# g1mv/density

Hardware: NVIDIA H100
Metric: chameleon_encode_input_GBps (higher is better)
Workload: dtype u32

## Files before the change

density_b200/csrc/api.cu:

```cuda
#include "../../include/density_b200.h"
#include "common.cuh"
#include "encode_internal.cuh"
#include "decode_bounds.cuh"

#include <dlfcn.h>

#include <atomic>
#include <condition_variable>
#include <cstdio>
#include <cstring>
#include <deque>
#include <mutex>
#include <string>
#include <thread>
#include <vector>

namespace dns {

static thread_local std::string g_last_error;
static std::atomic<uint64_t> g_launches{0};

static void set_error(const char* what, cudaError_t e) {
    char buf[512];
    snprintf(buf, sizeof buf, "%s: %s (%s)", what, cudaGetErrorString(e), cudaGetErrorName(e));
// ... 118 lines not shown
        ring.used[k] = true;
    }
    return e;
}
static cudaError_t d2h_any(PinRing& ring, uint8_t* dst, const uint8_t* src_dev, size_t n, cudaStream_t s, bool pageable) {
    if (!pageable) return cudaMemcpyAsync(dst, src_dev, n, cudaMemcpyDeviceToHost, s);
    cudaError_t e = ring.ensure();
    size_t pend_off = 0, pend_len = 0; unsigned pend_k = 0; bool pending = false;
    for (size_t off = 0; off < n && e == cudaSuccess; off += PIN_SLOT) {
        const size_t len = n - off < PIN_SLOT ? n - off : PIN_SLOT;
        const unsigned k = ring.next++ & 1u;
        if (ring.used[k] && !(pending && pend_k == k)) e = cudaEventSynchronize(ring.ev[k]);
        if (e != cudaSuccess) break;
        e = cudaMemcpyAsync(ring.slot[k], src_dev + off, len, cudaMemcpyDeviceToHost, s);
        if (e == cudaSuccess) e = cudaEventRecord(ring.ev[k], s);
        ring.used[k] = true;
        if (pending && e == cudaSuccess) {
            e = cudaEventSynchronize(ring.ev[pend_k]);
            if (e == cudaSuccess) CopyPool::get().copy(dst + pend_off, ring.slot[pend_k], pend_len);
        }
        pend_off = off; pend_len = len; pend_k = k; pending = true;
    }
    if (pending && e == cudaSuccess) {
        e = cudaEventSynchronize(ring.ev[pend_k]);
        if (e == cudaSuccess) CopyPool::get().copy(dst + pend_off, ring.slot[pend_k], pend_len);
    }
    return e;
}

struct DeviceCtx {
    int dev = -1;
    int num_sms = 0;
    bool ready = false;
    cudaStream_t stream = nullptr;
    cudaStream_t h2d_stream = nullptr, d2h_stream = nullptr;
    DevBuf ws, stage_in, stage_out, pipe_tables, dec_tables;
    DevBuf chee_tables[2][3];
    uint32_t chee_epoch = 0;
    uint64_t* h_sizes = nullptr;
    cudaEvent_t ev_h2d[2] = {nullptr, nullptr};
    PinRing ring_in, ring_out;
    uint64_t* d_size = nullptr;
    uint64_t* h_size = nullptr;
    ChamLayout layout{};
    int last_was_chameleon_fastpath_capable = 0;
    bool profile = false;
    static constexpr int PROF_RING = 64;
    cudaEvent_t ev[PROF_RING][4] = {};
    uint64_t prof_count = 0;
    const void* last_cl_status = nullptr;
    DevBuf lion_stats; bool lion_stats_valid = false;
    cudaEvent_t ws_free = nullptr;
    bool ws_free_recorded = false;
    std::mutex mu;
};

constexpr int MAX_DEVICES = 64;
static DeviceCtx g_ctx[MAX_DEVICES];
static std::mutex g_ctx_mu;

static DeviceCtx* current_ctx() {
    int dev = -1;
    cudaError_t e = cudaGetDevice(&dev);
    if (e != cudaSuccess) { set_error("cudaGetDevice", e); return nullptr; }
    if (dev < 0 || dev >= MAX_DEVICES) { set_error("device index out of range"); return nullptr; }
    DeviceCtx* c = &g_ctx[dev];
    std::lock_guard<std::mutex> lk(g_ctx_mu);
    if (!c->ready) {
        cudaDeviceProp prop;
        e = cudaGetDeviceProperties(&prop, dev);
        if (e != cudaSuccess) { set_error("cudaGetDeviceProperties", e); return nullptr; }
        if (prop.major != 9 || prop.minor != 0) { set_error("density_b200 is built for sm_90a and requires a compute capability 9.0 device (H100)"); return nullptr; }
        c->dev = dev;
        c->num_sms = prop.multiProcessorCount;
        e = cudaStreamCreateWithFlags(&c->stream, cudaStreamNonBlocking);
        if (e == cudaSuccess) e = cudaStreamCreateWithFlags(&c->h2d_stream, cudaStreamNonBlocking);
        if (e == cudaSuccess) e = cudaStreamCreateWithFlags(&c->d2h_stream, cudaStreamNonBlocking);
        if (e != cudaSuccess) { set_error("cudaStreamCreate", e); return nullptr; }
        e = cudaMalloc(&c->d_size, 64);
        if (e != cudaSuccess) { set_error("cudaMalloc", e); return nullptr; }
        e = cudaMallocHost(&c->h_size, 64);
        if (e == cudaSuccess) e = cudaMallocHost(&c->h_sizes, sizeof(uint64_t) * 4096);
        if (e != cudaSuccess) { set_error("cudaMallocHost", e); return nullptr; }
        e = cudaEventCreateWithFlags(&c->ws_free, cudaEventDisableTiming);
        if (e != cudaSuccess) { set_error("cudaEventCreate", e); return nullptr; }
        c->ready = true;
    }
    return c;
}

static size_t safe_size(int alg, size_t size) {
    const size_t B = alg_block_bytes(alg), S = alg_sig_bytes(alg);
    return size + (size / B) * S + ((size % B) ? S : 0);
}

static bool is_device_pointer(const void* p) {
    cudaPointerAttributes a;
    cudaError_t e = cudaPointerGetAttributes(&a, p);
    if (e != cudaSuccess) { cudaGetLastError(); return false; }
    return a.type == cudaMemoryTypeDevice || a.type == cudaMemoryTypeManaged;
}

static bool ws_acquire(DeviceCtx* c, cudaStream_t stream) {
    if (!c->ws_free_recorded) return true;
    cudaError_t e = cudaStreamWaitEvent(stream, c->ws_free, 0);
    if (e != cudaSuccess) { set_error("cudaStreamWaitEvent", e); return false; }
    return true;
}
static void ws_release(DeviceCtx* c, cudaStream_t stream) {
    if (cudaEventRecord(c->ws_free, stream) == cudaSuccess) c->ws_free_recorded = true;
}

static int encode_device_locked_impl(DeviceCtx* c, int alg, const uint8_t* d_in, size_t n, uint8_t* d_out, size_t cap,
                                     uint64_t* d_out_size, cudaStream_t stream, int path);
static int encode_device_locked(DeviceCtx* c, int alg, const uint8_t* d_in, size_t n, uint8_t* d_out, size_t cap,
                                uint64_t* d_out_size, cudaStream_t stream, int path) {
    if (!ws_acquire(c, stream)) return DENSITY_B200_ECUDA;
    const int rc = encode_device_locked_impl(c, alg, d_in, n, d_out, cap, d_out_size, stream, path);
    ws_release(c, stream);
    return rc;
}
static int encode_device_locked_impl(DeviceCtx* c, int alg, const uint8_t* d_in, size_t n, uint8_t* d_out, size_t cap,
                                     uint64_t* d_out_size, cudaStream_t stream, int path) {
    uint64_t launches = 0;
    cudaError_t e;
    const bool aligned = !(reinterpret_cast<uintptr_t>(d_in) & 3) && !(reinterpret_cast<uintptr_t>(d_out) & 1);
    if (alg == ALG_CHAMELEON && path != 3 && aligned) {
        ChamLayout L;
        size_t need = cham_workspace_bytes(n, c->num_sms, &L);
        e = c->ws.ensure(need, stream);
        if (e != cudaSuccess) { set_error("workspace cudaMalloc", e); return DENSITY_B200_ECUDA; }
        c->layout = L;
        if (path == 2) {
            e = cham_encode_protected_only(d_in, n, c->ws.p, L, d_out, cap, d_out_size, stream, &launches);
        } else {
            const uint32_t nruns = cham_pick_runs(n, c->num_sms);
            cudaEvent_t* ev = nullptr;
            if (c->profile) {
                ev = c->ev[c->prof_count % DeviceCtx::PROF_RING];
                for (int i = 0; i < 4; ++i) if (!ev[i]) cudaEventCreate(&ev[i]);
            }
            e = cham_encode_phase1(d_in, n, c->ws.p, L, nruns, nullptr, stream, &launches, ev);
            if (e == cudaSuccess && path == 4)
                e = cham_encode_phase2_blocking(d_in, n, c->ws.p, L, nruns, d_out, cap, d_out_size, 12, c->num_sms, stream, &launches);
            else if (e == cudaSuccess)
                e = cham_encode_phase2(d_in, n, c->ws.p, L, nruns, nullptr, d_out, cap, d_out_size, path == 0, false, c->num_sms, stream, &launches, ev);
            if (ev != nullptr && e == cudaSuccess) c->prof_count++;
        }
        c->last_was_chameleon_fastpath_capable = (path != 2);
    } else if ((alg == ALG_CHEETAH || alg == ALG_LION) && path != 3 && !(reinterpret_cast<uintptr_t>(d_in) & 3) && !(reinterpret_cast<uintptr_t>(d_out) & 1)) {
        const size_t pw = (chee_workspace_bytes(n, c->num_sms) + 255) & ~(size_t)255;
        e = c->ws.ensure(pw + 256 + scalar_workspace_bytes(alg), stream);
        if (e != cudaSuccess) { set_error("workspace cudaMalloc", e); return DENSITY_B200_ECUDA; }
        DevBuf* tb = c->chee_tables[alg == ALG_LION];
        for (int rg = 0; rg < 3 && e == cudaSuccess; ++rg) e = tb[rg].ensure(chee_tables_bytes(alg, rg, n, c->num_sms) + 256, stream);
        if (e != cudaSuccess) { set_error("workspace cudaMalloc", e); return DENSITY_B200_ECUDA; }
        if (c->chee_epoch > 0x0FFFFF00u) {
            for (int a2 = 0; a2 < 2; ++a2) for (int rg = 0; rg < 3; ++rg)
                if (c->chee_tables[a2][rg].p) { e = cudaMemsetAsync(c->chee_tables[a2][rg].p, 0, c->chee_tables[a2][rg].bytes, stream); if (e != cudaSuccess) break; }
            if (e != cudaSuccess) { set_error("cudaMemsetAsync", e); return DENSITY_B200_ECUDA; }
            c->chee_epoch = 0;
        }
        uint32_t* d_conv = reinterpret_cast<uint32_t*>(c->ws.p + pw);
        uint8_t* const tabs[3] = {tb[0].p, tb[1].p, tb[2].p};
        for (int attempt = 0; attempt <= (path == 4 ? 12 : 0); ++attempt) {
            if (attempt > 0) {
                uint32_t conv = 0;
                e = cudaMemcpyAsync(&conv, d_conv, sizeof conv, cudaMemcpyDeviceToHost, stream);
                if (e == cudaSuccess) e = cudaStreamSynchronize(stream);
                if (e != cudaSuccess || conv) break;
            }
            const uint32_t epoch_base = c->chee_epoch + 1;
            c->chee_epoch += 32;
            e = chee_encode_parallel(alg, d_in, n, d_out, cap, c->ws.p, tabs, epoch_base, c->num_sms, d_out_size, d_conv, attempt > 0, stream, &launches);
            if (e != cudaSuccess) break;
        }
        if (e == cudaSuccess && path != 1)
            e = scalar_encode(alg, d_in, n, d_out, cap, c->ws.p + pw + 256, d_out_size, stream, &launches, d_conv);
        c->last_was_chameleon_fastpath_capable = 0;
    } else {
        if (reinterpret_cast<uintptr_t>(d_out) & 1) { set_error("encode_device: d_out must be 2-byte aligned"); return DENSITY_B200_EARG; }
        e = c->ws.ensure(scalar_workspace_bytes(alg), stream);
        if (e != cudaSuccess) { set_error("workspace cudaMalloc", e); return DENSITY_B200_ECUDA; }
        e = scalar_encode(alg, d_in, n, d_out, cap, c->ws.p, d_out_size, stream, &launches);
        c->last_was_chameleon_fastpath_capable = 0;
    }
    return step_result(e, launches, "encode launch");
}

static int decode_device_locked_impl(DeviceCtx* c, int alg, const uint8_t* d_in, size_t n, uint8_t* d_out, size_t cap,
                                     uint64_t* d_out_size, cudaStream_t stream, int path);
static int decode_device_locked(DeviceCtx* c, int alg, const uint8_t* d_in, size_t n, uint8_t* d_out, size_t cap,
                                uint64_t* d_out_size, cudaStream_t stream, int path = 0) {
    if (!ws_acquire(c, stream)) return DENSITY_B200_ECUDA;
    const int rc = decode_device_locked_impl(c, alg, d_in, n, d_out, cap, d_out_size, stream, path);
    ws_release(c, stream);
    return rc;
}
static int decode_device_locked_impl(DeviceCtx* c, int alg, const uint8_t* d_in, size_t n, uint8_t* d_out, size_t cap,
// ... 1993 lines not shown
```

density_b200/csrc/chameleon_encode.cu:

```cuda
#include <cstdio>
#include "common.cuh"
#include "encode_internal.cuh"

namespace dns {
namespace cham {

constexpr int TILE_Q = 4096;
__device__ __forceinline__ bool bit_test(const uint32_t* bm, uint32_t i) { return (bm[i >> 5] >> (i & 31)) & 1u; }

constexpr int F6_THREADS = 512, F6_QPT = 8;
constexpr int F6_NW = F6_THREADS / 32, F6_WQ = 32 * F6_QPT;
static_assert(F6_THREADS * F6_QPT == TILE_Q, "tile geometry");
constexpr int F6_MB_SLOTS = 4096, F6_MB_CAP = 4;
constexpr int F6_SEC_SLOTS = 64, F6_SEC_CAP = 16;
#ifdef DNS_PHASE_TIMING
__device__ long long g_f6_ph[8];
#define F6_PH(k) { if (threadIdx.x == 0 && blockIdx.x == 77) { long long tn = clock64(); g_f6_ph[k] += tn - f6_tprev; f6_tprev = tn; } }
#define F6_PH_DECL long long f6_tprev = clock64();
#else
#define F6_PH(k)
#define F6_PH_DECL
#endif
constexpr uint32_t F6_TOUCHED = 1u << 12, F6_DROPPED = 1u << 13;
struct Flag6Smem {
    uint16_t tab[65536];
    uint32_t vbit[2048];
    uint2 rec[TILE_Q];
    union {
        uint16_t mb[F6_MB_SLOTS][F6_MB_CAP];
        uint2 stage[F6_NW][64];
    };
    uint32_t mbcnt[2][F6_MB_SLOTS / 4];
    __align__(16) uint32_t sec[F6_SEC_SLOTS][F6_SEC_CAP];
    uint32_t seccnt[2][F6_SEC_SLOTS];
    uint32_t sigw[2][TILE_Q / 32];
    uint32_t cnt[32];
    uint32_t unres_count;
    uint32_t overflow;
};
static_assert(sizeof(Flag6Smem) <= 227 * 1024, "flag pass shared memory");

__device__ __forceinline__ void f6_append_unres(bool pred, uint32_t qidx_in_run, uint32_t hf, uint32_t* s_count, uint2* __restrict__ unres_run) {
    const uint32_t m = __ballot_sync(0xFFFFFFFFu, pred);
    if (m == 0) return;
    uint32_t base = 0;
    if ((threadIdx.x & 31) == 0) base = atomicAdd(s_count, (uint32_t)__popc(m));
    base = __shfl_sync(0xFFFFFFFFu, base, 0);
    if (pred) {
        const uint32_t idx = base + __popc(m & lanemask_lt());
        if (idx < 65536u) unres_run[idx] = make_uint2(qidx_in_run, hf);
    }
}

// ... 1048 lines not shown
    for (uint32_t g = 0; g < ngrp; ++g) { gin[g] = x; if (x != PC_ESC) x = GT[(size_t)g * PC_NC + x]; }
    gin[ngrp] = x;
    if (x == PC_ESC) words[1] = 1;
}
__global__ void cham_prot_seams_k(uint32_t nseg, const Status* __restrict__ st, const uint16_t* __restrict__ T, const uint32_t* __restrict__ gin,
                                  uint32_t* __restrict__ in_state) {
    if (!gate_open(st)) return;
    const uint32_t ngrp = (nseg + PC_GROUP - 1) / PC_GROUP;
    const uint32_t g = blockIdx.x * blockDim.x + threadIdx.x;
    if (g >= ngrp || gin[ngrp] == PC_ESC) return;
    uint32_t x = gin[g];
    const uint32_t s1 = ((g + 1) * PC_GROUP < nseg) ? (g + 1) * PC_GROUP : nseg;
    for (uint32_t s = g * PC_GROUP; s < s1; ++s) { in_state[s] = x; x = T[(size_t)s * PC_NC + x]; }
}
__global__ void cham_prot_walk_k(uint64_t nblocks, uint32_t nseg, const Status* __restrict__ st, int it, int warm, const uint8_t* __restrict__ inc,
                                 const uint8_t* __restrict__ cm_old, uint8_t* __restrict__ cm_new, const uint32_t* __restrict__ in_state,
                                 const uint32_t* __restrict__ gin, ProtShard* __restrict__ ps, uint32_t* __restrict__ words) {
    if (!gate_open(st)) return;
    const uint32_t ngrp = (nseg + PC_GROUP - 1) / PC_GROUP;
    const uint32_t s = blockIdx.x * blockDim.x + threadIdx.x;
    if (s >= nseg || gin[ngrp] == PC_ESC) return;
    Protection p; pc_decode(in_state[s], p);
    const uint64_t b0 = (uint64_t)s * PSEG, b1 = (b0 + PSEG < nblocks) ? b0 + PSEG : nblocks;
    p.counter = ps->first_block + b0;
    prot_walk(p, inc, b0, b1, cm_new);
    uint32_t nd = 0;
    for (uint64_t b = b0; b < b1; ++b) nd += cm_new[b] != ((it || warm) ? cm_old[b] : 0);
    if (nd) {
        atomicAdd(&words[0], nd);
        if (it < 16) atomicAdd(&ps->changed[it], nd);
    }
}

__device__ __forceinline__ void prot_round_verdict(const uint32_t* all_words, uint32_t world, uint32_t stride, bool& changed, bool& esc) {
    changed = false; esc = false;
    for (uint32_t r = 0; r < world; ++r) { changed |= all_words[stride * r] != 0; esc |= all_words[stride * r + 1] != 0; }
}
__global__ void cham_prot_commit_k(const uint32_t* __restrict__ all_words, uint32_t world, uint32_t stride, uint64_t nblocks, const Status* __restrict__ st,
                                   int it, uint8_t* __restrict__ cm_old, const uint8_t* __restrict__ cm_new) {
    if (!gate_open(st)) return;
    bool changed, esc;
    prot_round_verdict(all_words, world, stride, changed, esc);
    if (esc || !(changed || it == 0)) return;
    for (uint64_t b = (uint64_t)blockIdx.x * blockDim.x + threadIdx.x; b < nblocks; b += (uint64_t)gridDim.x * blockDim.x) cm_old[b] = cm_new[b];
}
__global__ void cham_prot_verdict_k(const uint32_t* __restrict__ all_words, uint32_t world, uint32_t stride, Status* __restrict__ st, int it,
                                    ProtShard* __restrict__ ps) {
    if (threadIdx.x || blockIdx.x || !gate_open(st)) return;
    bool changed, esc;
    prot_round_verdict(all_words, world, stride, changed, esc);
    if (esc) { ps->esc = 1; st->converged = 1; }
    else if (!changed) { ps->settled = 1; ps->rounds = (uint32_t)it + 1; st->converged = 1; }
}
__global__ void cham_prot_finish_k(Status* __restrict__ st, const ProtShard* __restrict__ ps) {
    if (threadIdx.x || blockIdx.x) return;
    if (!ps->settled || !ps->stage_ok) st->error = PROT_REFUSED;
}
__global__ void cham_prot_seam_words_k(uint64_t nblocks, const Status* __restrict__ st, uint64_t* __restrict__ d_out_size, uint32_t* __restrict__ words) {
    if (threadIdx.x || blockIdx.x) return;
    const uint64_t sz = (nblocks && !st->error) ? *d_out_size : 0;
    *d_out_size = sz;
    words[0] = 0; words[1] = 0; words[2] = st->error ? 1u : 0u; words[3] = nblocks ? 1u : 0u;
    words[4] = (uint32_t)sz; words[5] = (uint32_t)(sz >> 32); words[6] = 0; words[7] = 0;
}

}

using namespace cham;

size_t cham_workspace_bytes(size_t nbytes, int nruns_max, ChamLayout* L) {
    const uint64_t nblocks = (nbytes + 255) / 256;
    const uint64_t ntiles = (nblocks + 63) / 64;
    const uint64_t ngroups = (ntiles + SCAN_G - 1) / SCAN_G;
    size_t off = 0;
    auto take = [&](size_t bytes) { size_t o = off; off += (bytes + 255) & ~(size_t)255; return o; };
    L->status = take(sizeof(Status));
    L->sigw = take((ntiles * 64 * 2 + 64 + 256) * sizeof(uint32_t));
    L->copymap = take(ntiles * 64 + 64 + 128);
    L->copymap2 = take(ntiles * 64 + 64 + 128);
    L->seg_state = take(prot_state_bytes(ntiles * 64 / PSEG + 2));
    L->incb = take(ntiles * 64 + 64);
    L->tile_bytes = take((ntiles + 1) * sizeof(uint32_t));
    L->tile_local = take((ntiles + 1) * sizeof(uint32_t));
    L->group_total = take((ngroups + 1) * sizeof(uint64_t));
    L->group_off = take((ngroups + 1) * sizeof(uint64_t));
    L->unres = take((size_t)nruns_max * 65536 * sizeof(uint2));
    L->unres_count = take((size_t)nruns_max * sizeof(uint32_t));
    L->final_tab = take((size_t)nruns_max * 65536 * sizeof(uint32_t));
    L->carry = take((size_t)nruns_max * 65536 * sizeof(uint32_t));
    L->total = off;
    return off;
}

static cudaError_t set_smem_attrs_once() {
    static bool done = false;
    static cudaError_t err = cudaSuccess;
    if (!done) {
        err = cudaFuncSetAttribute(cham_flag_pass6, cudaFuncAttributeMaxDynamicSharedMemorySize, (int)sizeof(Flag6Smem));
        if (err == cudaSuccess)
            err = cudaFuncSetAttribute(cham_protected_pass, cudaFuncAttributeMaxDynamicSharedMemorySize, (int)sizeof(ProtSmem));
        done = true;
    }
    return err;
}

static cudaError_t prot_iterate_coop(int ctas, cudaStream_t stream, const uint32_t* sigw, uint64_t nbytes, uint64_t nblocks, uint32_t nseg, Status* st, int it,
// ... 4 lines not shown

cudaError_t prot_debug_read(unsigned long long* out32) { return cudaMemcpyFromSymbol(out32, g_prot_dbg, sizeof(unsigned long long) * 32); }

size_t prot_state_bytes(uint64_t nseg_max) { return (2 * (nseg_max + 2) + 64) * sizeof(uint32_t) + prot_table_elems(nseg_max) * sizeof(uint16_t); }

uint32_t cham_pick_runs(size_t nbytes, int num_sms) {
    const uint64_t nblocks = (nbytes + 255) / 256;
    const uint64_t ntiles = (nblocks + 63) / 64;
    uint64_t r = ntiles / 16;
    if (r < 1) r = 1;
    if (r > (uint64_t)num_sms) r = num_sms;
    return (uint32_t)r;
}

struct ChamBufs {
    size_t nbytes; uint64_t nquads, nblocks; uint32_t ntiles, ngroups, nseg, ngrp;
    Status* st; uint32_t* sigw; uint8_t *copymap, *copymap2, *incb; uint32_t *seg_state, *tile_bytes, *tile_local; uint64_t *group_total, *group_off;
    uint2* unres; uint32_t *unres_count, *final_tab, *carry;
    uint32_t *in_state, *out_state, *gin; uint16_t *ptab, *T, *GT;
    template <class X> static X* at(uint8_t* ws, size_t off) { return reinterpret_cast<X*>(ws + off); }
    ChamBufs(uint8_t* ws, const ChamLayout& L, size_t n) {
        nbytes = n; nquads = n / 4; nblocks = (n + 255) / 256;
        ntiles = (uint32_t)((nblocks + 63) / 64); ngroups = (ntiles + SCAN_G - 1) / SCAN_G;
        nseg = (uint32_t)((nblocks + PSEG - 1) / PSEG); ngrp = (nseg + PC_GROUP - 1) / PC_GROUP;
        st = at<Status>(ws, L.status); sigw = at<uint32_t>(ws, L.sigw);
        copymap = ws + L.copymap; copymap2 = ws + L.copymap2; incb = ws + L.incb;
        seg_state = at<uint32_t>(ws, L.seg_state);
        tile_bytes = at<uint32_t>(ws, L.tile_bytes); tile_local = at<uint32_t>(ws, L.tile_local);
        group_total = at<uint64_t>(ws, L.group_total); group_off = at<uint64_t>(ws, L.group_off);
        unres = at<uint2>(ws, L.unres); unres_count = at<uint32_t>(ws, L.unres_count);
        final_tab = at<uint32_t>(ws, L.final_tab); carry = at<uint32_t>(ws, L.carry);
        in_state = seg_state; out_state = seg_state + (nseg + 1);
        ptab = reinterpret_cast<uint16_t*>(seg_state + 2 * (nseg + 1));
        gin = reinterpret_cast<uint32_t*>(ptab); T = ptab + 2 * (ngrp + 2); GT = T + (size_t)nseg * PC_NC;
    }
};

static void launch_flag_pass(const ChamBufs& B, const uint8_t* d_in, uint32_t nruns, const uint8_t* copymap, const Status* gate, cudaStream_t stream,
                             uint64_t* launches) {
    cham_flag_pass6<<<nruns, F6_THREADS, sizeof(Flag6Smem), stream>>>(reinterpret_cast<const uint32_t*>(d_in), B.nquads, B.ntiles, nruns, B.sigw, B.unres,
                                                                      B.unres_count, B.final_tab, copymap, gate);
    ++*launches;
}
static void launch_carry_resolve(const ChamBufs& B, uint32_t nruns, const uint32_t* d_carry_in, const Status* gate, cudaStream_t stream,
                                 uint64_t* launches) {
    cham_carry_scan<<<65536 / 256, 256, 0, stream>>>(B.final_tab, d_carry_in, 0, nruns, B.carry, nullptr, gate);
    cham_resolve<<<dim3(32, nruns), 256, 0, stream>>>(B.unres, B.unres_count, B.carry, B.ntiles, nruns, B.sigw, gate);
    *launches += 2;
}
static void launch_export_fold(const ChamBufs& B, uint32_t nruns, uint32_t* d_table_out, const Status* gate, cudaStream_t stream, uint64_t* launches) {
    cham_carry_scan<<<65536 / 256, 256, 0, stream>>>(B.final_tab, nullptr, 1, nruns, nullptr, d_table_out, gate);
    ++*launches;
}
static cudaError_t sizes_scan_emit(const ChamBufs& B, const uint8_t* d_in, const uint8_t* copymap, int use_copymap_if_nonquiet, bool al16_ok,
                                   uint8_t* d_out, size_t cap, uint64_t* d_out_size, cudaStream_t stream, uint64_t* launches, cudaEvent_t* ev) {
    if (copymap) {
        cham_tile_sizes<<<(B.ntiles + 7) / 8, 256, 0, stream>>>(B.sigw, copymap, B.nbytes, B.nblocks, B.ntiles, use_copymap_if_nonquiet, 0, 0, B.st, B.tile_bytes);
        ++*launches;
    }
    cudaError_t e = scan_tiles_launch(B.tile_bytes, B.ntiles, B.tile_local, B.group_total, B.group_off, B.ngroups, B.st, (uint64_t)cap, d_out_size, stream);
    if (e != cudaSuccess) return e;
    *launches += 2;
    if (ev) cudaEventRecord(ev[2], stream);
    const uint32_t* in32 = reinterpret_cast<const uint32_t*>(d_in);
    if (al16_ok && (reinterpret_cast<uintptr_t>(d_in) & 15u) == 0)
        cham_emit<true><<<B.ntiles, EM_THREADS, 0, stream>>>(in32, B.nbytes, B.nblocks, B.sigw, copymap, use_copymap_if_nonquiet, B.st, B.tile_local, B.group_off, d_out);
    else
        cham_emit<false><<<B.ntiles, EM_THREADS, 0, stream>>>(in32, B.nbytes, B.nblocks, B.sigw, copymap, use_copymap_if_nonquiet, B.st, B.tile_local, B.group_off, d_out);
    ++*launches;
    if (ev) cudaEventRecord(ev[3], stream);
    return cudaGetLastError();
}

cudaError_t cham_encode_phase1(const uint8_t* d_in, size_t nbytes, uint8_t* ws, const ChamLayout& L, uint32_t nruns,
                               uint32_t* d_table_out, cudaStream_t stream, uint64_t* launches, cudaEvent_t* ev) {
    cudaError_t e = set_smem_attrs_once();
    if (e != cudaSuccess) return e;
    const ChamBufs B(ws, L, nbytes);
    e = cudaMemsetAsync(B.st, 0, sizeof(Status), stream);
    if (e == cudaSuccess) e = cudaMemsetAsync(&B.st->first_nonquiet_block, 0xFF, sizeof(unsigned long long), stream);
    if (e != cudaSuccess) return e;
    if (B.nblocks == 0) return cudaSuccess;
    if (ev) cudaEventRecord(ev[0], stream);
    launch_flag_pass(B, d_in, nruns, nullptr, nullptr, stream, launches);
    if (ev) cudaEventRecord(ev[1], stream);
    if (d_table_out) launch_export_fold(B, nruns, d_table_out, nullptr, stream, launches);
    return cudaGetLastError();
}

static cudaError_t cham_phase2_begin(const ChamBufs& B, uint32_t nruns, const uint32_t* d_carry_in, bool assume_prev_inc, cudaStream_t stream,
                                     uint64_t* launches) {
    launch_carry_resolve(B, nruns, d_carry_in, nullptr, stream, launches);
    cham_tile_sizes<<<(B.ntiles + 7) / 8, 256, 0, stream>>>(B.sigw, nullptr, B.nbytes, B.nblocks, B.ntiles, 0, 1, assume_prev_inc ? 1 : 0, B.st, B.tile_bytes);
    ++*launches;
    return cudaGetLastError();
}

static cudaError_t cham_phase2_rounds(const ChamBufs& B, const uint8_t* d_in, uint32_t nruns, const uint32_t* d_carry_in, int it_first, int it_last,
                                      bool reset_barriers, int num_sms, cudaStream_t stream, uint64_t* launches) {
    const int num_ctas = num_sms > 0 ? num_sms : 1;
    if (it_last - it_first >= 8) return cudaErrorInvalidValue;
    if (reset_barriers) {
        cudaError_t e = cudaMemsetAsync(B.st->barrier, 0, sizeof(B.st->barrier), stream);
        if (e != cudaSuccess) return e;
    }
    for (int it = it_first; it <= it_last; ++it) {
        if (it > 0) {
            launch_flag_pass(B, d_in, nruns, B.copymap, B.st, stream, launches);
            launch_carry_resolve(B, nruns, d_carry_in, B.st, stream, launches);
        }
        cudaError_t le = prot_iterate_coop(num_ctas, stream, B.sigw, B.nbytes, B.nblocks, B.nseg, B.st, it, B.incb, B.copymap, B.copymap2, B.in_state,
                                           B.out_state, B.ptab);
        if (le != cudaSuccess) return le;
        ++*launches;
    }
    return cudaGetLastError();
}

static cudaError_t cham_phase2_finish(const ChamBufs& B, const uint8_t* d_in, uint8_t* d_out, size_t cap, uint64_t* d_out_size, bool with_copy_map,
                                      bool inorder_fallback, cudaStream_t stream, uint64_t* launches, cudaEvent_t* ev) {
    if (with_copy_map && inorder_fallback) {
        cham_protected_pass<<<1, 1024, sizeof(ProtSmem), stream>>>(reinterpret_cast<const uint32_t*>(d_in), B.nbytes, B.st, 1, B.sigw, B.copymap);
        ++*launches;
    }
    return sizes_scan_emit(B, d_in, with_copy_map ? B.copymap : nullptr, 1, true, d_out, cap, d_out_size, stream, launches, ev);
}

static cudaError_t cham_phase2_needs_more(const ChamBufs& B, cudaStream_t stream, bool* more) {
    Status h;
    cudaError_t e = cudaMemcpyAsync(&h, B.st, sizeof h, cudaMemcpyDeviceToHost, stream);
    if (e == cudaSuccess) e = cudaStreamSynchronize(stream);
    if (e != cudaSuccess) return e;
    *more = h.nonquiet && !h.converged && !h.error;
    return cudaSuccess;
}

constexpr int PROT_ITERS = 4;

struct Phase2Opts {
    const uint32_t* d_carry_in = nullptr;
    bool assume_prev_inc = false;
    bool iterate = true;
    int max_batches = 0;
    bool inorder_walk = true;
    bool* give_up = nullptr;
    uint32_t* d_table_out = nullptr;
    cudaEvent_t* ev = nullptr;
};

static cudaError_t cham_phase2(const uint8_t* d_in, size_t nbytes, uint8_t* ws, const ChamLayout& L, uint32_t nruns, uint8_t* d_out, size_t cap,
                               uint64_t* d_out_size, const Phase2Opts& o, int num_sms, cudaStream_t stream, uint64_t* launches) {
    if (nbytes == 0) return cudaMemsetAsync(d_out_size, 0, sizeof(uint64_t), stream);
    const ChamBufs B(ws, L, nbytes);
    cudaError_t e = cham_phase2_begin(B, nruns, o.d_carry_in, o.assume_prev_inc, stream, launches);
    if (e == cudaSuccess && o.iterate) e = cham_phase2_rounds(B, d_in, nruns, o.d_carry_in, 0, PROT_ITERS, false, num_sms, stream, launches);
    bool more = false;
    const int looks = o.max_batches + (o.give_up ? 1 : 0);
    for (int batch = 0; e == cudaSuccess && batch < looks; ++batch) {
        e = cham_phase2_needs_more(B, stream, &more);
        if (e != cudaSuccess || !more || batch >= o.max_batches) break;
        e = cham_phase2_rounds(B, d_in, nruns, o.d_carry_in, 8, 15, true, num_sms, stream, launches);
    }
    if (e != cudaSuccess) return e;
    if (o.give_up && more) { *o.give_up = true; return cudaSuccess; }
    e = cham_phase2_finish(B, d_in, d_out, cap, d_out_size, o.iterate, o.inorder_walk, stream, launches, o.ev);
    if (e == cudaSuccess && o.d_table_out) {
        launch_export_fold(B, nruns, o.d_table_out, nullptr, stream, launches);
        e = cudaGetLastError();
    }
    return e;
}

cudaError_t cham_encode_phase2(const uint8_t* d_in, size_t nbytes, uint8_t* ws, const ChamLayout& L, uint32_t nruns,
                               const uint32_t* d_carry_in, uint8_t* d_out, size_t cap, uint64_t* d_out_size,
                               bool allow_protected_fallback, bool assume_prev_inc, int num_sms, cudaStream_t stream, uint64_t* launches,
                               cudaEvent_t* ev) {
    Phase2Opts o;
    o.d_carry_in = d_carry_in; o.assume_prev_inc = assume_prev_inc; o.iterate = allow_protected_fallback; o.ev = ev;
    return cham_phase2(d_in, nbytes, ws, L, nruns, d_out, cap, d_out_size, o, num_sms, stream, launches);
}

cudaError_t cham_encode_phase2_blocking(const uint8_t* d_in, size_t nbytes, uint8_t* ws, const ChamLayout& L, uint32_t nruns, uint8_t* d_out,
                                        size_t cap, uint64_t* d_out_size, int max_batches, int num_sms, cudaStream_t stream, uint64_t* launches) {
    Phase2Opts o;
    o.max_batches = max_batches;
    return cham_phase2(d_in, nbytes, ws, L, nruns, d_out, cap, d_out_size, o, num_sms, stream, launches);
}

cudaError_t cham_encode_phase2_stream(const uint8_t* d_in, size_t nbytes, uint8_t* ws, const ChamLayout& L, uint32_t nruns, const uint32_t* d_carry_in,
                                      uint8_t* d_out, size_t cap, uint64_t* d_out_size, uint32_t* d_table_out, int max_batches, int num_sms,
                                      cudaStream_t stream, uint64_t* launches, bool* ok) {
    bool gave_up = false;
    Phase2Opts o;
    o.d_carry_in = d_carry_in; o.max_batches = max_batches; o.inorder_walk = false; o.give_up = &gave_up; o.d_table_out = d_table_out;
    const cudaError_t e = cham_phase2(d_in, nbytes, ws, L, nruns, d_out, cap, d_out_size, o, num_sms, stream, launches);
    *ok = !gave_up;
    return e;
}
cudaError_t cham_quads_to_table(const uint32_t* d_quads, uint32_t* d_table, cudaStream_t stream, uint64_t* launches) {
    cham_quads_to_table_k<<<65536 / 256, 256, 0, stream>>>(d_quads, d_table);
    ++*launches;
    return cudaGetLastError();
}
cudaError_t cham_table_into_quads(const uint32_t* d_table, uint32_t* d_quads, cudaStream_t stream, uint64_t* launches) {
    cham_table_into_quads_k<<<65536 / 256, 256, 0, stream>>>(d_table, d_quads);
    ++*launches;
    return cudaGetLastError();
}

cudaError_t cham_status_accumulate(const uint8_t* ws, const ChamLayout& L, uint32_t* d_flag, cudaStream_t stream, uint64_t* launches) {
    cham_status_accumulate_k<<<1, 1, 0, stream>>>(reinterpret_cast<const Status*>(ws + L.status), d_flag);
    ++*launches;
    return cudaGetLastError();
}
cudaError_t prot_iterate_launch(const uint32_t* sigw_or_null, uint64_t nbytes, uint64_t nblocks, uint32_t nseg, Status* st, int it, uint8_t* inc,
                                uint8_t* cm_old, uint8_t* cm_new, uint32_t* in_state, uint32_t* out_state, int num_sms, cudaStream_t stream) {
    int ctas = num_sms > 0 ? num_sms : 1;
    if ((uint32_t)ctas > nseg) ctas = nseg ? (int)nseg : 1;
    return prot_iterate_coop(ctas, stream, sigw_or_null, nbytes, nblocks, nseg, st, it, inc, cm_old, cm_new, in_state, out_state,
                             reinterpret_cast<uint16_t*>(out_state + (nseg + 1)));
}
cudaError_t scan_tiles_launch(const uint32_t* tile_bytes, uint32_t ntiles, uint32_t* tile_local, uint64_t* group_total, uint64_t* group_off,
                              uint32_t ngroups, Status* st, uint64_t cap, uint64_t* d_out_size, cudaStream_t stream) {
    scan_groups_local<<<ngroups, SCAN_T, 0, stream>>>(tile_bytes, ntiles, tile_local, group_total);
    scan_group_totals<<<1, SCAN_T, 0, stream>>>(group_total, ngroups, group_off, st, cap, d_out_size);
    return cudaGetLastError();
}
cudaError_t cham_rank_fold(const uint32_t* d_tables, uint32_t rank, uint32_t* d_carry, cudaStream_t stream, uint64_t* launches) {
    cham_rank_fold_k<<<65536 / 256, 256, 0, stream>>>(d_tables, rank, d_carry);
    ++*launches;
    return cudaGetLastError();
}
cudaError_t cham_seam_words(const uint8_t* ws, const ChamLayout& L, size_t nbytes, const uint64_t* d_out_size, uint32_t* d_words, cudaStream_t stream, uint64_t* launches) {
    cham_seam_words_k<<<1, 1, 0, stream>>>(reinterpret_cast<const uint32_t*>(ws + L.sigw), nbytes, (nbytes + 255) / 256,
                                           reinterpret_cast<const Status*>(ws + L.status), d_out_size, d_words);
    ++*launches;
    return cudaGetLastError();
}
cudaError_t cham_seam_verdict(const uint32_t* d_all_words, uint32_t world, uint32_t rank, uint32_t* d_flags, uint64_t* d_total, uint64_t* d_offsets,
                              cudaStream_t stream, uint64_t* launches) {
    cham_seam_verdict_k<<<1, 1, 0, stream>>>(d_all_words, world, rank, d_flags, d_total, d_offsets);
    ++*launches;
    return cudaGetLastError();
}
cudaError_t cham_table_init(uint32_t* d_table, cudaStream_t stream, uint64_t* launches) {
    cham_table_init_k<<<65536 / 256, 256, 0, stream>>>(d_table);
    ++*launches;
    return cudaGetLastError();
}
cudaError_t cham_table_fold(uint32_t* d_acc, const uint32_t* d_next, cudaStream_t stream, uint64_t* launches) {
    cham_table_fold_k<<<65536 / 256, 256, 0, stream>>>(d_acc, d_next);
    ++*launches;
    return cudaGetLastError();
}

cudaError_t cham_encode_protected_only(const uint8_t* d_in, size_t nbytes, uint8_t* ws, const ChamLayout& L, uint8_t* d_out,
                                       size_t cap, uint64_t* d_out_size, cudaStream_t stream, uint64_t* launches) {
    cudaError_t e = set_smem_attrs_once();
    if (e != cudaSuccess) return e;
    const ChamBufs B(ws, L, nbytes);
    e = cudaMemsetAsync(B.st, 0, sizeof(Status), stream);
    if (e != cudaSuccess) return e;
    if (B.nblocks == 0) return cudaMemsetAsync(d_out_size, 0, sizeof(uint64_t), stream);
    cham_protected_pass<<<1, 1024, sizeof(ProtSmem), stream>>>(reinterpret_cast<const uint32_t*>(d_in), nbytes, B.st, 0, B.sigw, B.copymap);
    ++*launches;
    return sizes_scan_emit(B, d_in, B.copymap, 0, false, d_out, cap, d_out_size, stream, launches, nullptr);
}

ProtSegs prot_segs(Status* st, uint64_t nbytes, uint64_t nblocks, uint8_t* inc, uint8_t* cm, uint8_t* cm2, uint32_t* seg_state) {
    ProtSegs P;
    P.st = st; P.nbytes = nbytes; P.nblocks = nblocks; P.inc = inc; P.cm = cm; P.cm2 = cm2;
    P.nseg = (uint32_t)((nblocks + PSEG - 1) / PSEG); P.ngrp = (P.nseg + PC_GROUP - 1) / PC_GROUP;
    P.in_state = seg_state;
    uint16_t* ptab = reinterpret_cast<uint16_t*>(seg_state + 2 * (P.nseg + 1));
    P.gin = reinterpret_cast<uint32_t*>(ptab); P.T = ptab + 2 * (P.ngrp + 2); P.GT = P.T + (size_t)P.nseg * PC_NC;
    return P;
}
cudaError_t prot_start(const ProtSegs& P, ProtShard* ps, uint64_t first_block, const uint64_t* d_lengths, uint32_t rank, uint32_t block_bytes,
                       cudaStream_t stream, uint64_t* launches) {
    cham_prot_start_k<<<1, 32, 0, stream>>>(P.st, ps, first_block, d_lengths, rank, block_bytes);
    ++*launches;
    return cudaGetLastError();
}
cudaError_t prot_transfer(const ProtSegs& P, const uint32_t* sigw, const ProtShard* ps, int it, uint32_t* d_transfer_out, cudaStream_t stream,
                          uint64_t* launches) {
    if (P.nblocks) {
        cham_prot_seg_k<<<P.nseg < 2048u ? P.nseg : 2048u, PSEG, 0, stream>>>(sigw, P.nbytes, P.nblocks, P.nseg, P.st, it, P.inc, P.cm, ps, P.T);
        cham_prot_groups_k<<<(P.ngrp * PC_NC + 255) / 256, 256, 0, stream>>>(P.nseg, P.st, P.T, P.GT);
        *launches += 2;
    }
    cham_prot_transfer_k<<<1, 256, 0, stream>>>(P.nseg, P.st, P.GT, d_transfer_out);
    ++*launches;
    return cudaGetLastError();
}
cudaError_t prot_settle(const ProtSegs& P, ProtShard* ps, int it, int warm, const uint32_t* d_all_transfers, uint32_t rank, uint32_t* d_words,
                        cudaStream_t stream, uint64_t* launches) {
    cham_prot_enter_k<<<1, 32, 0, stream>>>(d_all_transfers, rank, P.nseg, P.st, P.GT, P.gin, ps, d_words);
    ++*launches;
    if (P.nseg) {
        cham_prot_seams_k<<<(P.ngrp + 127) / 128, 128, 0, stream>>>(P.nseg, P.st, P.T, P.gin, P.in_state);
        cham_prot_walk_k<<<(P.nseg + 127) / 128, 128, 0, stream>>>(P.nblocks, P.nseg, P.st, it, warm, P.inc, P.cm, P.cm2, P.in_state, P.gin, ps, d_words);
        *launches += 2;
    }
    return cudaGetLastError();
}
cudaError_t prot_commit(const ProtSegs& P, ProtShard* ps, int it, const uint32_t* d_all_words, uint32_t world, uint32_t stride, cudaStream_t stream,
                        uint64_t* launches) {
    if (P.nblocks) {
        cham_prot_commit_k<<<(uint32_t)((P.nblocks + 1023) / 1024 < 1024 ? (P.nblocks + 1023) / 1024 : 1024), 256, 0, stream>>>(
            d_all_words, world, stride, P.nblocks, P.st, it, P.cm, P.cm2);
        ++*launches;
    }
    cham_prot_verdict_k<<<1, 32, 0, stream>>>(d_all_words, world, stride, P.st, it, ps);
    ++*launches;
    return cudaGetLastError();
}
cudaError_t prot_refuse_unsettled(Status* st, const ProtShard* ps, cudaStream_t stream, uint64_t* launches) {
    cham_prot_finish_k<<<1, 32, 0, stream>>>(st, ps);
    ++*launches;
// ... 65 lines not shown
```

density_b200/csrc/encode_internal.cuh:

```cuda
#pragma once
#include <cuda_runtime.h>
#include <stdint.h>
#include <stddef.h>

namespace dns {

struct ChamLayout {
    size_t status, sigw, copymap, copymap2, seg_state, incb, tile_bytes, tile_local, group_total, group_off, unres, unres_count, final_tab, carry, total;
};

size_t cham_workspace_bytes(size_t nbytes, int nruns_max, ChamLayout* L);
uint32_t cham_pick_runs(size_t nbytes, int num_sms);
cudaError_t cham_encode_phase1(const uint8_t* d_in, size_t nbytes, uint8_t* ws, const ChamLayout& L, uint32_t nruns,
                               uint32_t* d_table_out, cudaStream_t stream, uint64_t* launches, cudaEvent_t* ev = nullptr);
cudaError_t cham_encode_phase2(const uint8_t* d_in, size_t nbytes, uint8_t* ws, const ChamLayout& L, uint32_t nruns,
                               const uint32_t* d_carry_in, uint8_t* d_out, size_t cap, uint64_t* d_out_size,
                               bool allow_protected_fallback, bool assume_prev_inc, int num_sms, cudaStream_t stream, uint64_t* launches,
                               cudaEvent_t* ev = nullptr);
cudaError_t cham_encode_phase2_blocking(const uint8_t* d_in, size_t nbytes, uint8_t* ws, const ChamLayout& L, uint32_t nruns, uint8_t* d_out,
                                        size_t cap, uint64_t* d_out_size, int max_batches, int num_sms, cudaStream_t stream, uint64_t* launches);
cudaError_t cham_encode_protected_only(const uint8_t* d_in, size_t nbytes, uint8_t* ws, const ChamLayout& L, uint8_t* d_out,
                                       size_t cap, uint64_t* d_out_size, cudaStream_t stream, uint64_t* launches);

cudaError_t cham_quads_to_table(const uint32_t* d_quads, uint32_t* d_table, cudaStream_t stream, uint64_t* launches);
cudaError_t cham_table_into_quads(const uint32_t* d_table, uint32_t* d_quads, cudaStream_t stream, uint64_t* launches);
cudaError_t cham_encode_phase2_stream(const uint8_t* d_in, size_t nbytes, uint8_t* ws, const ChamLayout& L, uint32_t nruns, const uint32_t* d_carry_in,
                                      uint8_t* d_out, size_t cap, uint64_t* d_out_size, uint32_t* d_table_out, int max_batches, int num_sms,
                                      cudaStream_t stream, uint64_t* launches, bool* ok);

cudaError_t cham_status_accumulate(const uint8_t* ws, const ChamLayout& L, uint32_t* d_flag, cudaStream_t stream, uint64_t* launches);
cudaError_t cham_table_init(uint32_t* d_table, cudaStream_t stream, uint64_t* launches);
cudaError_t cham_rank_fold(const uint32_t* d_tables, uint32_t rank, uint32_t* d_carry, cudaStream_t stream, uint64_t* launches);
cudaError_t cham_seam_words(const uint8_t* ws, const ChamLayout& L, size_t nbytes, const uint64_t* d_out_size, uint32_t* d_words, cudaStream_t stream, uint64_t* launches);
cudaError_t cham_seam_verdict(const uint32_t* d_all_words, uint32_t world, uint32_t rank, uint32_t* d_flags, uint64_t* d_total, uint64_t* d_offsets,
                              cudaStream_t stream, uint64_t* launches);
cudaError_t cham_table_fold(uint32_t* d_acc, const uint32_t* d_next, cudaStream_t stream, uint64_t* launches);

struct Status;
size_t prot_state_bytes(uint64_t nseg_max);
cudaError_t prot_debug_read(unsigned long long* out32);
cudaError_t prot_iterate_launch(const uint32_t* sigw_or_null, uint64_t nbytes, uint64_t nblocks, uint32_t nseg, Status* st, int it, uint8_t* inc,
                                uint8_t* cm_old, uint8_t* cm_new, uint32_t* in_state, uint32_t* out_state, int num_sms, cudaStream_t stream);
cudaError_t scan_tiles_launch(const uint32_t* tile_bytes, uint32_t ntiles, uint32_t* tile_local, uint64_t* group_total, uint64_t* group_off,
                              uint32_t ngroups, Status* st, uint64_t cap, uint64_t* d_out_size, cudaStream_t stream);

struct ProtShard {
    unsigned long long first_block;
    uint32_t rounds;
    uint32_t settled, in_state, esc;
    uint32_t changed[16];
    uint32_t stage_ok;
    uint32_t has_quad, last_quad;
};
constexpr uint32_t PROT_TRANSFER_WORDS = 200, PROT_ROUND_WORDS = 4, PROT_MAX_ROUNDS = 16;
struct ProtSegs {
    Status* st; uint64_t nbytes, nblocks; uint32_t nseg, ngrp;
    uint8_t *inc, *cm, *cm2; uint32_t *in_state, *gin; uint16_t *T, *GT;
};
ProtSegs prot_segs(Status* st, uint64_t nbytes, uint64_t nblocks, uint8_t* inc, uint8_t* cm, uint8_t* cm2, uint32_t* seg_state);
cudaError_t prot_start(const ProtSegs& P, ProtShard* ps, uint64_t first_block, const uint64_t* d_lengths, uint32_t rank, uint32_t block_bytes,
                       cudaStream_t stream, uint64_t* launches);
cudaError_t prot_transfer(const ProtSegs& P, const uint32_t* sigw, const ProtShard* ps, int it, uint32_t* d_transfer_out, cudaStream_t stream,
                          uint64_t* launches);
cudaError_t prot_settle(const ProtSegs& P, ProtShard* ps, int it, int warm, const uint32_t* d_all_transfers, uint32_t rank, uint32_t* d_words,
                        cudaStream_t stream, uint64_t* launches);
cudaError_t prot_commit(const ProtSegs& P, ProtShard* ps, int it, const uint32_t* d_all_words, uint32_t world, uint32_t stride, cudaStream_t stream,
                        uint64_t* launches);
cudaError_t prot_refuse_unsettled(Status* st, const ProtShard* ps, cudaStream_t stream, uint64_t* launches);
cudaError_t prot_seam_words(uint64_t nblocks, Status* st, uint64_t* d_out_size, uint32_t* d_seam8, cudaStream_t stream, uint64_t* launches);
cudaError_t cham_prot_start(uint8_t* ws, const ChamLayout& L, ProtShard* ps, uint64_t first_block, const uint64_t* d_lengths, uint32_t rank,
                            cudaStream_t stream, uint64_t* launches);
// ... 113 lines not shown
```

Measured before the change: 484.3.

## Wrap chameleon phase-2 protected rounds in cached conditional CUDA graph

Captures the protected-fallback rounds and settle kernels into a CUDA graph with an IF conditional node. The node is gated on a device-side status flag (nonquiet), so the whole tail is skipped on device when no fallback is needed. The instantiated graph is cached per context and keyed on buffer pointers, layout and sizes. This replaces the many individual launches of the iterative rounds, which otherwise queue up even when their kernels early-exit. In exchange it costs a graph build whenever the inputs change, and it depends on conditional-node support, with a fallback to the old path if the build fails.

```diff
diff --git a/density_b200/csrc/api.cu b/density_b200/csrc/api.cu
--- a/density_b200/csrc/api.cu
+++ b/density_b200/csrc/api.cu
@@ -194,6 +194,7 @@
     DevBuf lion_stats; bool lion_stats_valid = false;
     cudaEvent_t ws_free = nullptr;
     bool ws_free_recorded = false;
+    ChamTailGraph tail;
     std::mutex mu;
 };
 
@@ -286,7 +287,8 @@
             if (e == cudaSuccess && path == 4)
                 e = cham_encode_phase2_blocking(d_in, n, c->ws.p, L, nruns, d_out, cap, d_out_size, 12, c->num_sms, stream, &launches);
             else if (e == cudaSuccess)
-                e = cham_encode_phase2(d_in, n, c->ws.p, L, nruns, nullptr, d_out, cap, d_out_size, path == 0, false, c->num_sms, stream, &launches, ev);
+                e = cham_encode_phase2(d_in, n, c->ws.p, L, nruns, nullptr, d_out, cap, d_out_size, path == 0, false, c->num_sms, stream, &launches, ev,
+                                       &c->tail);
             if (ev != nullptr && e == cudaSuccess) c->prof_count++;
         }
         c->last_was_chameleon_fastpath_capable = (path != 2);
diff --git a/density_b200/csrc/chameleon_encode.cu b/density_b200/csrc/chameleon_encode.cu
--- a/density_b200/csrc/chameleon_encode.cu
+++ b/density_b200/csrc/chameleon_encode.cu
@@ -1,4 +1,6 @@
 #include <cstdio>
+#include <cstdlib>
+#include <cstring>
 #include "common.cuh"
 #include "encode_internal.cuh"
 
@@ -1153,6 +1155,10 @@
     if (esc) { ps->esc = 1; st->converged = 1; }
     else if (!changed) { ps->settled = 1; ps->rounds = (uint32_t)it + 1; st->converged = 1; }
 }
+__global__ void cham_tail_condition_k(cudaGraphConditionalHandle h, const Status* __restrict__ st) {
+    if (threadIdx.x || blockIdx.x) return;
+    cudaGraphSetConditional(h, st->nonquiet ? 1u : 0u);
+}
 __global__ void cham_prot_finish_k(Status* __restrict__ st, const ProtShard* __restrict__ ps) {
     if (threadIdx.x || blockIdx.x) return;
     if (!ps->settled || !ps->stage_ok) st->error = PROT_REFUSED;
@@ -1263,12 +1269,12 @@
     cham_carry_scan<<<65536 / 256, 256, 0, stream>>>(B.final_tab, nullptr, 1, nruns, nullptr, d_table_out, gate);
     ++*launches;
 }
-static cudaError_t sizes_scan_emit(const ChamBufs& B, const uint8_t* d_in, const uint8_t* copymap, int use_copymap_if_nonquiet, bool al16_ok,
-                                   uint8_t* d_out, size_t cap, uint64_t* d_out_size, cudaStream_t stream, uint64_t* launches, cudaEvent_t* ev) {
-    if (copymap) {
-        cham_tile_sizes<<<(B.ntiles + 7) / 8, 256, 0, stream>>>(B.sigw, copymap, B.nbytes, B.nblocks, B.ntiles, use_copymap_if_nonquiet, 0, 0, B.st, B.tile_bytes);
-        ++*launches;
-    }
+static void launch_copymap_sizes(const ChamBufs& B, const uint8_t* copymap, int use_copymap_if_nonquiet, cudaStream_t stream, uint64_t* launches) {
+    cham_tile_sizes<<<(B.ntiles + 7) / 8, 256, 0, stream>>>(B.sigw, copymap, B.nbytes, B.nblocks, B.ntiles, use_copymap_if_nonquiet, 0, 0, B.st, B.tile_bytes);
+    ++*launches;
+}
+static cudaError_t scan_emit(const ChamBufs& B, const uint8_t* d_in, const uint8_t* copymap, int use_copymap_if_nonquiet, bool al16_ok,
+                             uint8_t* d_out, size_t cap, uint64_t* d_out_size, cudaStream_t stream, uint64_t* launches, cudaEvent_t* ev) {
     cudaError_t e = scan_tiles_launch(B.tile_bytes, B.ntiles, B.tile_local, B.group_total, B.group_off, B.ngroups, B.st, (uint64_t)cap, d_out_size, stream);
     if (e != cudaSuccess) return e;
     *launches += 2;
@@ -1328,13 +1334,18 @@
     return cudaGetLastError();
 }
 
+static void cham_phase2_settle(const ChamBufs& B, const uint8_t* d_in, bool inorder_fallback, cudaStream_t stream, uint64_t* launches) {
+    if (inorder_fallback) {
+        cham_protected_pass<<<1, 1024, sizeof(ProtSmem), stream>>>(reinterpret_cast<const uint32_t*>(d_in), B.nbytes, B.st, 1, B.sigw, B.copymap);
+        ++*launches;
+    }
+    launch_copymap_sizes(B, B.copymap, 1, stream, launches);
+}
+
 static cudaError_t cham_phase2_finish(const ChamBufs& B, const uint8_t* d_in, uint8_t* d_out, size_t cap, uint64_t* d_out_size, bool with_copy_map,
                                       bool inorder_fallback, cudaStream_t stream, uint64_t* launches, cudaEvent_t* ev) {
-    if (with_copy_map && inorder_fallback) {
-        cham_protected_pass<<<1, 1024, sizeof(ProtSmem), stream>>>(reinterpret_cast<const uint32_t*>(d_in), B.nbytes, B.st, 1, B.sigw, B.copymap);
-        ++*launches;
-    }
-    return sizes_scan_emit(B, d_in, with_copy_map ? B.copymap : nullptr, 1, true, d_out, cap, d_out_size, stream, launches, ev);
+    if (with_copy_map) cham_phase2_settle(B, d_in, inorder_fallback, stream, launches);
+    return scan_emit(B, d_in, with_copy_map ? B.copymap : nullptr, 1, true, d_out, cap, d_out_size, stream, launches, ev);
 }
 
 static cudaError_t cham_phase2_needs_more(const ChamBufs& B, cudaStream_t stream, bool* more) {
@@ -1347,6 +1358,70 @@
 }
 
 constexpr int PROT_ITERS = 4;
+
+static cudaError_t tail_graph_build(ChamTailGraph& T, const ChamBufs& B, const uint8_t* d_in, uint32_t nruns, const uint32_t* d_carry_in,
+                                    int num_sms, cudaGraphExec_t* exec, uint64_t* body_launches) {
+    cudaError_t e = T.capture ? cudaSuccess : cudaStreamCreateWithFlags(&T.capture, cudaStreamNonBlocking);
+    cudaGraph_t g = nullptr;
+    if (e == cudaSuccess) e = cudaGraphCreate(&g, 0);
+    if (e != cudaSuccess) return e;
+    cudaGraphConditionalHandle h = 0;
+    cudaGraphNode_t cond_node = nullptr, if_node = nullptr;
+    e = cudaGraphConditionalHandleCreate(&h, g, 0, 0);
+    if (e == cudaSuccess) {
+        const Status* st = B.st;
+        void* args[] = {&h, &st};
+        cudaKernelNodeParams kp = {};
+        kp.func = reinterpret_cast<void*>(cham_tail_condition_k);
+        kp.gridDim = dim3(1); kp.blockDim = dim3(32); kp.kernelParams = args;
+        e = cudaGraphAddKernelNode(&cond_node, g, nullptr, 0, &kp);
+    }
+    cudaGraphNodeParams np = {};
+    np.type = cudaGraphNodeTypeConditional;
+    np.conditional.handle = h; np.conditional.type = cudaGraphCondTypeIf; np.conditional.size = 1;
+    if (e == cudaSuccess) e = cudaGraphAddNode(&if_node, g, &cond_node, 1, &np);
+    if (e == cudaSuccess) e = cudaStreamBeginCaptureToGraph(T.capture, np.conditional.phGraph_out[0], nullptr, nullptr, 0, cudaStreamCaptureModeThreadLocal);
+    if (e == cudaSuccess) {
+        *body_launches = 0;
+        e = cham_phase2_rounds(B, d_in, nruns, d_carry_in, 0, PROT_ITERS, false, num_sms, T.capture, body_launches);
+        if (e == cudaSuccess) {
+            cham_phase2_settle(B, d_in, true, T.capture, body_launches);
+            e = cudaGetLastError();
+        }
+        cudaGraph_t body = nullptr;
+        const cudaError_t e2 = cudaStreamEndCapture(T.capture, &body);
+        if (e == cudaSuccess) e = e2;
+    }
+    cudaGraphExec_t x = nullptr;
+    if (e == cudaSuccess) e = cudaGraphInstantiate(&x, g, 0);
+    if (e == cudaSuccess) *exec = x;
+    cudaGraphDestroy(g);
+    return e;
+}
+
+static cudaError_t tail_graph_launch(ChamTailGraph& T, const ChamBufs& B, const uint8_t* ws, const ChamLayout& L, const uint8_t* d_in, uint32_t nruns,
+                                     const uint32_t* d_carry_in, int num_sms, cudaStream_t stream, uint64_t* launches, bool* launched) {
+    *launched = false;
+    const char* sw = getenv("DENSITY_B200_TAIL_GRAPH");
+    if (T.unavailable || (sw && strcmp(sw, "0") == 0)) return cudaSuccess;
+    const bool same = T.exec && T.ws == ws && memcmp(&T.L, &L, sizeof L) == 0 && T.d_in == d_in && T.d_carry_in == d_carry_in &&
+                      T.nbytes == B.nbytes && T.nruns == nruns && T.num_sms == num_sms;
+    if (!same) {
+        if (T.exec) cudaGraphExecDestroy(T.exec);
+        T.exec = nullptr;
+        if (tail_graph_build(T, B, d_in, nruns, d_carry_in, num_sms, &T.exec, &T.body_launches) != cudaSuccess) {
+            cudaGetLastError();
+            T.unavailable = true;
+            return cudaSuccess;
+        }
+        T.ws = ws; T.L = L; T.d_in = d_in; T.d_carry_in = d_carry_in; T.nbytes = B.nbytes; T.nruns = nruns; T.num_sms = num_sms;
+    }
+    const cudaError_t e = cudaGraphLaunch(T.exec, stream);
+    if (e != cudaSuccess) return e;
+    *launches += T.body_launches;
+    *launched = true;
+    return cudaSuccess;
+}
 
 struct Phase2Opts {
     const uint32_t* d_carry_in = nullptr;
@@ -1357,6 +1432,7 @@
     bool* give_up = nullptr;
     uint32_t* d_table_out = nullptr;
     cudaEvent_t* ev = nullptr;
+    ChamTailGraph* tail = nullptr;
 };
 
 static cudaError_t cham_phase2(const uint8_t* d_in, size_t nbytes, uint8_t* ws, const ChamLayout& L, uint32_t nruns, uint8_t* d_out, size_t cap,
@@ -1364,7 +1440,10 @@
     if (nbytes == 0) return cudaMemsetAsync(d_out_size, 0, sizeof(uint64_t), stream);
     const ChamBufs B(ws, L, nbytes);
     cudaError_t e = cham_phase2_begin(B, nruns, o.d_carry_in, o.assume_prev_inc, stream, launches);
-    if (e == cudaSuccess && o.iterate) e = cham_phase2_rounds(B, d_in, nruns, o.d_carry_in, 0, PROT_ITERS, false, num_sms, stream, launches);
+    bool tail_done = false;
+    if (e == cudaSuccess && o.tail && o.iterate && o.inorder_walk && o.max_batches == 0 && !o.give_up)
+        e = tail_graph_launch(*o.tail, B, ws, L, d_in, nruns, o.d_carry_in, num_sms, stream, launches, &tail_done);
+    if (e == cudaSuccess && o.iterate && !tail_done) e = cham_phase2_rounds(B, d_in, nruns, o.d_carry_in, 0, PROT_ITERS, false, num_sms, stream, launches);
     bool more = false;
     const int looks = o.max_batches + (o.give_up ? 1 : 0);
     for (int batch = 0; e == cudaSuccess && batch < looks; ++batch) {
@@ -1374,7 +1453,8 @@
     }
     if (e != cudaSuccess) return e;
     if (o.give_up && more) { *o.give_up = true; return cudaSuccess; }
-    e = cham_phase2_finish(B, d_in, d_out, cap, d_out_size, o.iterate, o.inorder_walk, stream, launches, o.ev);
+    e = tail_done ? scan_emit(B, d_in, B.copymap, 1, true, d_out, cap, d_out_size, stream, launches, o.ev)
+                  : cham_phase2_finish(B, d_in, d_out, cap, d_out_size, o.iterate, o.inorder_walk, stream, launches, o.ev);
     if (e == cudaSuccess && o.d_table_out) {
         launch_export_fold(B, nruns, o.d_table_out, nullptr, stream, launches);
         e = cudaGetLastError();
@@ -1385,9 +1465,9 @@
 cudaError_t cham_encode_phase2(const uint8_t* d_in, size_t nbytes, uint8_t* ws, const ChamLayout& L, uint32_t nruns,
                                const uint32_t* d_carry_in, uint8_t* d_out, size_t cap, uint64_t* d_out_size,
                                bool allow_protected_fallback, bool assume_prev_inc, int num_sms, cudaStream_t stream, uint64_t* launches,
-                               cudaEvent_t* ev) {
+                               cudaEvent_t* ev, ChamTailGraph* tail) {
     Phase2Opts o;
-    o.d_carry_in = d_carry_in; o.assume_prev_inc = assume_prev_inc; o.iterate = allow_protected_fallback; o.ev = ev;
+    o.d_carry_in = d_carry_in; o.assume_prev_inc = assume_prev_inc; o.iterate = allow_protected_fallback; o.ev = ev; o.tail = tail;
     return cham_phase2(d_in, nbytes, ws, L, nruns, d_out, cap, d_out_size, o, num_sms, stream, launches);
 }
 
@@ -1475,7 +1555,8 @@
     if (B.nblocks == 0) return cudaMemsetAsync(d_out_size, 0, sizeof(uint64_t), stream);
     cham_protected_pass<<<1, 1024, sizeof(ProtSmem), stream>>>(reinterpret_cast<const uint32_t*>(d_in), nbytes, B.st, 0, B.sigw, B.copymap);
     ++*launches;
-    return sizes_scan_emit(B, d_in, B.copymap, 0, false, d_out, cap, d_out_size, stream, launches, nullptr);
+    launch_copymap_sizes(B, B.copymap, 0, stream, launches);
+    return scan_emit(B, d_in, B.copymap, 0, false, d_out, cap, d_out_size, stream, launches, nullptr);
 }
 
 ProtSegs prot_segs(Status* st, uint64_t nbytes, uint64_t nblocks, uint8_t* inc, uint8_t* cm, uint8_t* cm2, uint32_t* seg_state) {
diff --git a/density_b200/csrc/encode_internal.cuh b/density_b200/csrc/encode_internal.cuh
--- a/density_b200/csrc/encode_internal.cuh
+++ b/density_b200/csrc/encode_internal.cuh
@@ -9,6 +9,15 @@
     size_t status, sigw, copymap, copymap2, seg_state, incb, tile_bytes, tile_local, group_total, group_off, unres, unres_count, final_tab, carry, total;
 };
 
+struct ChamTailGraph {
+    cudaGraphExec_t exec = nullptr;
+    cudaStream_t capture = nullptr;
+    bool unavailable = false;
+    uint64_t body_launches = 0;
+    const uint8_t* ws = nullptr; ChamLayout L{}; const uint8_t* d_in = nullptr; const uint32_t* d_carry_in = nullptr; size_t nbytes = 0;
+    uint32_t nruns = 0; int num_sms = 0;
+};
+
 size_t cham_workspace_bytes(size_t nbytes, int nruns_max, ChamLayout* L);
 uint32_t cham_pick_runs(size_t nbytes, int num_sms);
 cudaError_t cham_encode_phase1(const uint8_t* d_in, size_t nbytes, uint8_t* ws, const ChamLayout& L, uint32_t nruns,
@@ -16,7 +25,7 @@
 cudaError_t cham_encode_phase2(const uint8_t* d_in, size_t nbytes, uint8_t* ws, const ChamLayout& L, uint32_t nruns,
                                const uint32_t* d_carry_in, uint8_t* d_out, size_t cap, uint64_t* d_out_size,
                                bool allow_protected_fallback, bool assume_prev_inc, int num_sms, cudaStream_t stream, uint64_t* launches,
-                               cudaEvent_t* ev = nullptr);
+                               cudaEvent_t* ev = nullptr, ChamTailGraph* tail = nullptr);
 cudaError_t cham_encode_phase2_blocking(const uint8_t* d_in, size_t nbytes, uint8_t* ws, const ChamLayout& L, uint32_t nruns, uint8_t* d_out,
                                         size_t cap, uint64_t* d_out_size, int max_batches, int num_sms, cudaStream_t stream, uint64_t* launches);
 cudaError_t cham_encode_protected_only(const uint8_t* d_in, size_t nbytes, uint8_t* ws, const ChamLayout& L, uint8_t* d_out,
```

New measurement: 495.0 (median of 6 runs). 1.02x the previous value.
